# ascentai/diy-gym

Hardware: AMD Instinct MI355X
Metric: env steps/sec (whole node) (higher is better)
Workload: dtype f32; 1 GPU; ur_high_5 x 16384 envs per GPU; envs_total=16384, substeps=2, auto_reset=True, launch=hipGraph replay of 8-step segments, parallelism=independent env shards x1, no collective, envs_per_wavefront=64, lds_bytes_per_workgroup=160512, parity=vs the C oracle only; parity with pybullet itself is UNPINNED (DESIGN.md 4)

## Files before the change

### diy_gym_amd/csrc/dg_kernels.h

```cpp
#pragma once
#include "dg_device.h"
#include "../../include/diygym_scene.h"
#include "../../include/diygym_hip.h"

namespace dg {

#define DG_MAX_LINKS 64
#define DG_MAX_BODIES 192

#define DG_CONSTANT __attribute__((address_space(4)))
typedef const int32_t DG_CONSTANT* cip;
typedef const float DG_CONSTANT* cfp;

struct DevScene {
  cip BI, LI, FI, SI, PI, GI, OI, IL;
  cfp BF, LF, FF, SF, PF, OF, FL, HF;
  cip PLB;
  int split_pgs;
  int early_dyn;
  int coll_split, cont2_off;
  int coll_wave;
  cfp GD;
  cip AM;
  cip SD;
// ... 17 lines not shown
  int32_t reg_body[2];
  int32_t num_envs, stride;
  uint64_t seed; int64_t env_base;
  float h, gx, gy, gz;
  float hm;
};
struct MotorTable { float v[DG_MAX_LINKS * 3]; };

enum { PLB_R0 = 0, PLB_MINV, PLB_DV, PLB_NV, PLB_CHAIN , PLB_STRIDE };
enum { PLL_POSE = 0, PLL_MROW, PLL_IAACC , PLL_STRIDE };
enum { AW_E = 0, AW_R = 9, AW_V = 12, AW_PA = 18, AW_U = 24, AW_D = 30, AW_UU = 31, AW_STRIDE = 32 };
enum { AB_V = 0, AB_A = 6, AB_FIXED_STRIDE = 12, AB_IA = 12, AB_PA = 33, AB_L = 39, AB_FLOAT_STRIDE = 60 };
enum { CL_PAIR = 0, CL_P = 1, CL_N = 4, CL_DIST = 7, CL_KEY = 8, CL_DVA = 9, CL_NVA = 10, CL_DVB = 11, CL_NVB = 12, CL_MU = 13, CL_STRIDE = 14 };
enum { MR_B = 0, MR_ACC, MR_LO_B, MR_LO_ACC, MR_HI_B, MR_HI_ACC, MR_STRIDE };

constexpr int envs_per_wave(int lanes) { return lanes > 0 ? lanes : (lanes < 0 ? -lanes : 64); }

template <int LANES>
DGD float* workspace_of(const DevScene& sc, float* smem, float* gws, int lane) {
  if constexpr (LANES > 0) return smem + lane;
  else return gws + (size_t)blockIdx.x * (size_t)sc.total_slots * envs_per_wave(LANES) + lane;
}

template <int LANES>
struct Lane {
  const DevScene& sc;
  const MotorTable& mt;
  float* lds;
  float* st;
  int env;
  bool valid;

  DGD Lane(const DevScene& s, const MotorTable& m, float* l, float* state, int e, bool v) : sc(s), mt(m), lds(l), st(state), env(e), valid(v) {}

  DGD float& L(int slot) const { return lds[slot * envs_per_wave(LANES)]; }
  DGD float S(int k) const { return st[(size_t)k * sc.stride]; }
  DGD void Sset(int k, float v) const { if (valid) st[(size_t)k * sc.stride] = v; }

  DGD V3 L3(int o) const { return v3(L(o), L(o + 1), L(o + 2)); }
  DGD void L3set(int o, V3 v) const { L(o) = v.x; L(o + 1) = v.y; L(o + 2) = v.z; }
  DGD M3 LM(int o) const { M3 A; _Pragma("unroll") for (int k = 0; k < 9; k++) A.m[k] = L(o + k); return A; }
  DGD void LMset(int o, const M3& A) const { _Pragma("unroll") for (int k = 0; k < 9; k++) L(o + k) = A.m[k]; }
  DGD M3 LR(int o) const {
    V3 c0 = v3(L(o), L(o + 1), L(o + 2)), c1 = v3(L(o + 3), L(o + 4), L(o + 5)), c2 = cross(c0, c1);
    M3 R = {{c0.x, c1.x, c2.x, c0.y, c1.y, c2.y, c0.z, c1.z, c2.z}}; return R;
  }
// ... 37 lines not shown
  DGD V3 base_pos(int b) const {
    if (frozen(b)) { cfp f = bf(b) + DG_BF_INIT_POS; return v3(f[0], f[1], f[2]); }
    int o = bi(b)[DG_BI_STATE_OFF]; return v3(S(o), S(o + 1), S(o + 2));
  }
  DGD Q4 base_quat(int b) const {
    if (frozen(b)) { cfp f = bf(b) + DG_BF_INIT_QUAT; Q4 q = {f[0], f[1], f[2], f[3]}; return q; }
    int o = bi(b)[DG_BI_STATE_OFF] + DG_BS_QUAT; Q4 q = {S(o), S(o + 1), S(o + 2), S(o + 3)}; return q;
  }

  DGD void link_world(int b, int gl, M3& R, V3& p) const {
    if (gl < 0) { R = frozen(b) ? qmat(base_quat(b)) : LR(plb(b)[PLB_R0]); p = base_pos(b); }
    else { int o = pll(gl)[PLL_POSE]; R = LR(o); p = L3(o + 6); }
  }

  DGD void joint_xform(int gl, float q, M3& Rpc, V3& r) const {
    cfp f = lf(gl);
    M3 RT; _Pragma("unroll") for (int k = 0; k < 9; k++) RT.m[k] = f[DG_LF_ROT + k];
    V3 pT = v3(f[DG_LF_POS], f[DG_LF_POS + 1], f[DG_LF_POS + 2]);
    V3 ax = v3(f[DG_LF_AXIS], f[DG_LF_AXIS + 1], f[DG_LF_AXIS + 2]);
    if (li(gl)[DG_LI_TYPE] == 0) { Rpc = mul(RT, rot_axis(ax, q)); r = pT; }
    else { Rpc = RT; r = pT + mul(RT, ax * q); }
  }

  DGD void kinematics_chain(int b) const {
    constexpr int N = 6;
    cip B = bi(b); const int first = B[DG_BI_FIRST_LINK], n = B[DG_BI_N_LINKS];
    M3 R = qmat(base_quat(b)); V3 p = base_pos(b);
    LRset(plb(b)[PLB_R0], R);
    float qv[N];
#pragma unroll
    for (int j = 0; j < N; j++) qv[j] = S(li(first + min(j, n - 1))[DG_LI_STATE_OFF] + DG_LS_Q);
#pragma unroll
    for (int j = 0; j < N; j++) {
      if (j < n) {
        const int gl = first + j; M3 Rpc; V3 r; joint_xform(gl, qv[j], Rpc, r);
        const M3 Rn = mul(R, Rpc); p = p + mul(R, r);
        const int o = pll(gl)[PLL_POSE];
        LRset(o, Rn); L3set(o + 6, p);
        const V3 c0 = v3(Rn.m[0], Rn.m[3], Rn.m[6]), c1 = v3(Rn.m[1], Rn.m[4], Rn.m[7]), c2 = cross(c0, c1);
        const M3 Rb = {{c0.x, c1.x, c2.x, c0.y, c1.y, c2.y, c0.z, c1.z, c2.z}}; R = Rb;
      }
    }
  }
  DGD void kinematics(int b, int qoff = -1) const {
    cip B = bi(b);
    if (B[DG_BI_FLAGS] & DG_BODY_FROZEN) return;
    if (qoff < 0 && plb(b)[PLB_CHAIN]) { kinematics_chain(b); return; }
    int first = B[DG_BI_FIRST_LINK], n = B[DG_BI_N_LINKS];
    M3 R0 = qmat(base_quat(b)); V3 p0 = base_pos(b);
    LRset(plb(b)[PLB_R0], R0);
    constexpr int KCH = 8;
    for (int i0 = 0; i0 < n; i0 += KCH) {
      float qv[KCH];
#pragma unroll
      for (int j = 0; j < KCH; j++) { const int i = min(i0 + j, n - 1); qv[j] = qoff >= 0 ? L(qoff + i) : S(li(first + i)[DG_LI_STATE_OFF] + DG_LS_Q); }
#pragma unroll
      for (int j = 0; j < KCH; j++) {
        const int i = i0 + j; if (i >= n) break;
        int gl = first + i, par = li(gl)[DG_LI_PARENT];
        M3 Rpc; V3 r; joint_xform(gl, qv[j], Rpc, r);
        M3 Rp; V3 pp;
        if (par < 0) { Rp = R0; pp = p0; } else { int o = pll(par)[PLL_POSE]; Rp = LR(o); pp = L3(o + 6); }
        int o = pll(gl)[PLL_POSE];
        LRset(o, mul(Rp, Rpc)); L3set(o + 6, pp + mul(Rp, r));
// ... 191 lines not shown
        float rhs[6] = {-p0.a.x, -p0.a.y, -p0.a.z, -p0.l.x, -p0.l.y, -p0.l.z}, x[6];
        if (jdof < 0) {
#pragma unroll
          for (int k = 0; k < 6; k++) rhs[k] = (k == col) ? 1.0f : 0.0f;
        }
        chol6_solve(Lb, rhs, x);
        a0c.a = v3(x[0], x[1], x[2]); a0c.l = v3(x[3], x[4], x[5]);
#pragma unroll
        for (int k = 0; k < 6; k++) L(mo + col * nv + k) = x[k];
      }
      for (int i = 0; i <= jdof; i++) {
        int gl = first + i, par = li(gl)[DG_LI_PARENT]; int o = aw(i);
        S6 ap = par < 0 ? a0c : L6(aw(par - first) + AW_V);
        S6 a1 = xmotion(LM(o + AW_E), L3(o + AW_R), ap);
        float qdd = (L(o + AW_UU) - dot(L6(o + AW_U), a1)) / L(o + AW_D);
        L6set(o + AW_V, a1 + subspace(gl) * qdd);
        L(mo + col * nv + nb6 + i) = qdd;
      }
    }
    for (int r = 0; r < nv; r++) for (int c = r + 1; c < nv; c++) L(mo + r * nv + c) = L(mo + c * nv + r);
    prof.stamp(4 );
  }

  template <int N, class PROF_T>
  DGD void dynamics_chain(int b, PROF_T& prof) const {
    cip B = bi(b); const int first = B[DG_BI_FIRST_LINK], n = B[DG_BI_N_LINKS], mo = plb(b)[PLB_MINV]; const float h = sc.h;
    const M3 R0 = LR(plb(b)[PLB_R0]); const V3 gb = tmul(R0, v3(sc.gx, sc.gy, sc.gz));
    const float ka = ang_damping(b);
    const S6 zero6 = {v3(0.f, 0.f, 0.f), v3(0.f, 0.f, 0.f)};
    M3 E[N]; V3 r[N]; S6 v[N], pA[N], U[N], Sx[N]; float dinv[N], u[N], qd[N];
    S6 vp = zero6;
#pragma unroll
    for (int i = 0; i < N; i++) {
      E[i] = R0; r[i] = v3(0.f, 0.f, 0.f); v[i] = zero6; pA[i] = zero6; U[i] = zero6; Sx[i] = zero6; dinv[i] = 0.f; u[i] = 0.f; qd[i] = 0.f;
      if (i < n) {
        const int gl = first + i, lo = li(gl)[DG_LI_STATE_OFF]; cfp f = lf(gl);
        const float q = S(lo + DG_LS_Q); qd[i] = S(lo + DG_LS_QD);
        M3 Rpc; joint_xform(gl, q, Rpc, r[i]); E[i] = transpose(Rpc); Sx[i] = subspace(gl);
        v[i] = xmotion(E[i], r[i], vp) + Sx[i] * qd[i]; vp = v[i];
        float lm; V3 c; Sym3 Ic; link_inertia(gl, lm, c, Ic); (void)f;
        const AI I = rigid_inertia(lm, c, Ic);
        pA[i] = crf(v[i], mul(I, v[i])) - damping_force(lm, c, Ic, v[i], ka);
      }
    }
    AI carry; bool have = false;
#pragma unroll
    for (int i = N - 1; i >= 0; i--) {
      if (i < n) {
        const int gl = first + i, lo = li(gl)[DG_LI_STATE_OFF]; cfp f = lf(gl);
        const float tau = S(lo + DG_LS_TORQUE) - f[DG_LF_DAMPING] * qd[i];
        AI IA; { float lm; V3 lc; Sym3 lI; link_inertia(gl, lm, lc, lI); IA = rigid_inertia(lm, lc, lI); }
        if (have) {
          IA.I.xx += carry.I.xx; IA.I.xy += carry.I.xy; IA.I.xz += carry.I.xz; IA.I.yy += carry.I.yy; IA.I.yz += carry.I.yz; IA.I.zz += carry.I.zz;
          IA.M.xx += carry.M.xx; IA.M.xy += carry.M.xy; IA.M.xz += carry.M.xz; IA.M.yy += carry.M.yy; IA.M.yz += carry.M.yz; IA.M.zz += carry.M.zz;
#pragma unroll
          for (int k = 0; k < 9; k++) IA.H.m[k] += carry.H.m[k];
        }
        U[i] = mul(IA, Sx[i]); const float d = dot(Sx[i], U[i]); dinv[i] = 1.0f / d; u[i] = tau - dot(Sx[i], pA[i]);
        if (i > 0) {
          const float di = dinv[i]; const S6 Ui = U[i];
          AI Ia = IA;
          Ia.I.xx -= Ui.a.x * Ui.a.x * di; Ia.I.xy -= Ui.a.x * Ui.a.y * di; Ia.I.xz -= Ui.a.x * Ui.a.z * di;
          Ia.I.yy -= Ui.a.y * Ui.a.y * di; Ia.I.yz -= Ui.a.y * Ui.a.z * di; Ia.I.zz -= Ui.a.z * Ui.a.z * di;
          Ia.M.xx -= Ui.l.x * Ui.l.x * di; Ia.M.xy -= Ui.l.x * Ui.l.y * di; Ia.M.xz -= Ui.l.x * Ui.l.z * di;
          Ia.M.yy -= Ui.l.y * Ui.l.y * di; Ia.M.yz -= Ui.l.y * Ui.l.z * di; Ia.M.zz -= Ui.l.z * Ui.l.z * di;
          const float ua[3] = {Ui.a.x, Ui.a.y, Ui.a.z}, ul[3] = {Ui.l.x, Ui.l.y, Ui.l.z};
#pragma unroll
          for (int a = 0; a < 3; a++)
#pragma unroll
            for (int c2 = 0; c2 < 3; c2++) Ia.H.m[3 * a + c2] -= ua[a] * ul[c2] * di;
          const S6 c = crm(v[i], Sx[i] * qd[i]);
          const S6 pa = pA[i] + mul(Ia, c) + Ui * (u[i] * di);
          carry = to_parent(Ia, E[i], r[i]); have = true;
          pA[i - 1] = pA[i - 1] + xforce_to_parent(E[i], r[i], pa);
        }
      }
    }
    S6 ap; ap.a = v3(0.f, 0.f, 0.f); ap.l = -gb;
#pragma unroll
    for (int i = 0; i < N; i++) {
      if (i < n) {
        const S6 a1 = xmotion(E[i], r[i], ap) + crm(v[i], Sx[i] * qd[i]);
        const float qdd = (u[i] - dot(U[i], a1)) * dinv[i];
        ap = a1 + Sx[i] * qdd;
        Sset(li(first + i)[DG_LI_STATE_OFF] + DG_LS_QD, qd[i] + h * qdd);
      }
    }
    prof.stamp(3 );
#pragma unroll
    for (int col = 0; col < N; col++) {
      if (col < n) {
        S6 p[N]; float uu[N];
#pragma unroll
        for (int i = 0; i < N; i++) { p[i] = zero6; uu[i] = 0.f; }
#pragma unroll
        for (int i = col; i >= 0; i--) {
          uu[i] = (i == col ? 1.0f : 0.0f) - dot(Sx[i], p[i]);
          if (i > 0) p[i - 1] = p[i - 1] + xforce_to_parent(E[i], r[i], p[i] + U[i] * (uu[i] * dinv[i]));
        }
        S6 a = zero6;
#pragma unroll
        for (int i = 0; i < N; i++) {
          if (i < n) {
            const S6 a1 = xmotion(E[i], r[i], a);
            const float qdd = (uu[i] - dot(U[i], a1)) * dinv[i];
            a = a1 + Sx[i] * qdd;
            L(mo + col * n + i) = qdd;
          }
// ... 142 lines not shown
```

### diy_gym_amd/csrc/dg_solver.h

```cpp
#pragma once
#include "dg_kernels.h"
#include "dg_hull.h"

namespace dg {

enum { PS_UPDATE = 0, PS_KIN, PS_COLLIDE, PS_ABA, PS_MINV, PS_ROWS, PS_PGS, PS_INTEGRATE, PS_OUTPUT, PS_PGS_MOTOR, PS_PGS_LIMIT, PS_PGS_CONTACT, PS_COUNT,
       PS_ROW = PS_COUNT + 12  };
template <bool PROF> struct Prof;
template <> struct Prof<false> { DGD void start() {} DGD void stamp(int) {} };
template <> struct Prof<true> {
  unsigned long long last, acc[PS_COUNT];
  DGD void start() { _Pragma("unroll") for (int k = 0; k < PS_COUNT; k++) acc[k] = 0ull; last = __builtin_amdgcn_s_memtime(); }
  DGD void stamp(int id) {
    unsigned long long t = __builtin_amdgcn_s_memtime();
    _Pragma("unroll") for (int k = 0; k < PS_COUNT; k++) if (k == id) acc[k] += t - last;
    last = t;
  }
};

struct WShape { int type, body, glink; M3 R; V3 p; float prm0, prm1, prm2, mu; int poff, npts; };

template <int LANES>
DGD void shape_world(const Lane<LANES>& ln, int sh, WShape& o) {
  cip si = ln.sc.SI + sh * DG_SI_STRIDE; cfp sf = ln.sc.SF + sh * DG_SF_STRIDE;
// ... 1548 lines not shown
              const float mu = buf[d].mu;
              if (mu > 0.f) { const float lim = mu * buf[d].nacc; solve_row(buf[d], 3 * (t >> 1) + 1 + (t & 1), -lim, lim); }
            }
          }
        }
      }
    }
    prof.stamp(PS_PGS_CONTACT);
    if (live) iters_done = it + 1;
    live = live && !(maxres <= thr);
    if (!__any(live)) break;
  }
#pragma unroll
  for (int i = 0; i < NS; i++) if (i * SL + sl < nt) blk[(unsigned)(sc.dv_base + i * SL) * W + (lane_off >> 2)] = dv[i];
  if (sl == 0) for (int c = 0; c < ncont; c++) { _Pragma("unroll") for (int d = 0; d < 3; d++) blk[(unsigned)(r0 + (3 * c + d) * rs + 2 * nt + 1) * W + colq] = acc[(3 * c + d) * EPW]; }
  for (uint64_t m = rows.motors; m; m &= m - 1) {
    const int gl = __ffsll((long long)m) - 1; int col, mo, jg, base, nv; float lm; rows.get(gl, col, mo, jg, base, nv, lm);
    blk[(unsigned)(mo + MR_ACC) * W + colq] = acc[(3 * maxc + gl) * EPW];
  }
  return __shfl(iters_done, (lane << LOG) & 63);
}

template <int LANES>
DGD void setup_link_rows(const Lane<LANES>& ln, int g0, int g1, uint64_t& limit_mask, uint64_t& limit_rows) {
  const DevScene& sc = ln.sc; const float h = sc.h, lerp = sc.HF[DG_HF_LIMIT_ERP];
  constexpr int LCH = 6;
  for (int gc = g0; gc < g1; gc += LCH) {
    float q_[LCH], qd_[LCH], tp_[LCH], tv_[LCH];
#pragma unroll
    for (int j = 0; j < LCH; j++) {
      const int gl = min(gc + j, g1 - 1), lo = ln.li(gl)[DG_LI_STATE_OFF];
      q_[j] = ln.S(lo + DG_LS_Q); qd_[j] = ln.S(lo + DG_LS_QD); tp_[j] = ln.S(lo + DG_LS_TARGET_POS); tv_[j] = ln.S(lo + DG_LS_TARGET_VEL);
    }
#pragma unroll
    for (int j = 0; j < LCH; j++) {
      const int gl = gc + j; if (gl >= g1) break;
      const int mo = ln.pll(gl)[PLL_MROW]; cfp f = ln.lf(gl);
      const float q = q_[j], qd = qd_[j];
      const float kp = ln.mt.v[3 * gl], kd = ln.mt.v[3 * gl + 1];
      ln.L(mo + MR_B) = kp * (tp_[j] - q) / h + kd * (tv_[j] - qd);
      ln.L(mo + MR_ACC) = 0.f;
      const bool limited = f[DG_LF_LOWER] <= f[DG_LF_UPPER];
      const float dlo = q - f[DG_LF_LOWER], dhi = f[DG_LF_UPPER] - q;
      ln.L(mo + MR_LO_B) = -qd + (dlo > 0.f ? -dlo / h : -dlo * lerp / h); ln.L(mo + MR_LO_ACC) = (limited && dlo < 0.25f) ? 0.f : -1.f;
      ln.L(mo + MR_HI_B) = qd + (dhi > 0.f ? -dhi / h : -dhi * lerp / h); ln.L(mo + MR_HI_ACC) = (limited && dhi < 0.25f) ? 0.f : -1.f;
      if (__any(limited && (dlo < 0.25f || dhi < 0.25f))) limit_mask |= 1ull << (ln.li(gl)[DG_LI_BODY] & 63);
      if (gl < 32) { if (__any(limited && dlo < 0.25f)) limit_rows |= 1ull << (2 * gl); if (__any(limited && dhi < 0.25f)) limit_rows |= 2ull << (2 * gl); }
    }
  }
}

template <int LANES>
DGD void integrate_body(const Lane<LANES>& ln, int b) {
  const DevScene& sc = ln.sc; const float h = sc.h, vmax = sc.HF[DG_HF_MAX_COORD_VEL];
  constexpr int LCH = 6;
  cip B = ln.bi(b); const int n = B[DG_BI_N_LINKS], first = B[DG_BI_FIRST_LINK], so = B[DG_BI_STATE_OFF];
  const bool fx = ln.fixed(b); if (fx && n == 0) return;
  const int dvo = ln.plb(b)[PLB_DV];
  if (!fx) {
    M3 R0 = ln.LR(ln.plb(b)[PLB_R0]);
    V3 dw = mul(R0, ln.L3(dvo)), dl = mul(R0, ln.L3(dvo + 3));
    V3 w = v3(ln.S(so + DG_BS_ANGVEL), ln.S(so + DG_BS_ANGVEL + 1), ln.S(so + DG_BS_ANGVEL + 2)) + dw;
    V3 v = v3(ln.S(so + DG_BS_LINVEL), ln.S(so + DG_BS_LINVEL + 1), ln.S(so + DG_BS_LINVEL + 2)) + dl;
    ln.Sset(so + DG_BS_ANGVEL, w.x); ln.Sset(so + DG_BS_ANGVEL + 1, w.y); ln.Sset(so + DG_BS_ANGVEL + 2, w.z);
    ln.Sset(so + DG_BS_LINVEL, v.x); ln.Sset(so + DG_BS_LINVEL + 1, v.y); ln.Sset(so + DG_BS_LINVEL + 2, v.z);
    ln.Sset(so, ln.S(so) + h * v.x); ln.Sset(so + 1, ln.S(so + 1) + h * v.y); ln.Sset(so + 2, ln.S(so + 2) + h * v.z);
    float wn = norm(w), th = wn * h; Q4 dq;
    if (th > 1e-12f) { float sn, cs; sincosf(0.5f * th, &sn, &cs); sn /= wn; dq.x = w.x * sn; dq.y = w.y * sn; dq.z = w.z * sn; dq.w = cs; }
    else { dq.x = 0.5f * h * w.x; dq.y = 0.5f * h * w.y; dq.z = 0.5f * h * w.z; dq.w = 1.f; }
    Q4 qn = qnormalize(qmul(dq, ln.base_quat(b)));
    ln.Sset(so + 3, qn.x); ln.Sset(so + 4, qn.y); ln.Sset(so + 5, qn.z); ln.Sset(so + 6, qn.w);
  }
  const int k0 = fx ? 0 : 6;
  for (int i0 = 0; i0 < n; i0 += LCH) {
    float q_[LCH], qd_[LCH], dv_[LCH], ac_[LCH]; int lo_[LCH];
#pragma unroll
    for (int j = 0; j < LCH; j++) {
      const int i = min(i0 + j, n - 1); lo_[j] = ln.li(first + i)[DG_LI_STATE_OFF];
      q_[j] = ln.S(lo_[j] + DG_LS_Q); qd_[j] = ln.S(lo_[j] + DG_LS_QD); dv_[j] = ln.L(dvo + k0 + i); ac_[j] = ln.L(ln.pll(first + i)[PLL_MROW] + MR_ACC);
    }
#pragma unroll
    for (int j = 0; j < LCH; j++) {
      const int i = i0 + j; if (i >= n) break;
      const float maxf = ln.mt.v[3 * (first + i) + 2]; const float maximp = maxf < 0.f ? -maxf : maxf * sc.hm;
      ln.Sset(lo_[j] + DG_LS_APPLIED, maximp > 0.f ? ac_[j] / h : 0.f);
      const float qd = fminf(fmaxf(qd_[j] + dv_[j], -vmax), vmax);
      ln.Sset(lo_[j] + DG_LS_QD, qd); ln.Sset(lo_[j] + DG_LS_Q, q_[j] + h * qd);
    }
  }
}

#define DG_SPLIT_MAX_CONTACTS 3
DGD int split_slots(const DevScene& sc) { return sc.dv_base + sc.nt + sc.nv_max; }

template <int LANES>
DGD bool split_decide_main(const Lane<LANES>& ln, int wave_max_cont, uint64_t& limit_mask, uint64_t& limit_rows) {
  const DevScene& sc = ln.sc; const int xo = split_slots(sc);
  ln.L(xo + 4) = (sc.split_pgs && (wave_max_cont == 0 || (sc.split_pgs == 2 && wave_max_cont <= DG_SPLIT_MAX_CONTACTS))) ? 1.f : 0.f;
  __syncthreads();
  const unsigned hbits = (unsigned)ln.L(xo + 5);
  if (hbits) { limit_mask |= 1ull << (sc.helper_body & 63); limit_rows |= (uint64_t)hbits << (2 * ln.bi(sc.helper_body)[DG_BI_FIRST_LINK]); }
  return ln.L(xo + 4) != 0.f;
}
template <int LANES>
DGD bool split_decide_follow(const Lane<LANES>& ln, unsigned my_limit_bits, bool i_am_helper) {
  const DevScene& sc = ln.sc; const int xo = split_slots(sc);
  if (i_am_helper) ln.L(xo + 5) = (float)my_limit_bits;
  __syncthreads();
  return ln.L(xo + 4) != 0.f;
}

DGD float half_swap_max(float x) {
  float a = x, b = x;
  asm volatile("s_nop 1\n\tv_permlane32_swap_b32 %0, %1" : "+v"(a), "+v"(b));
// ... 125 lines not shown
        contact_row(3 * c + 1, -lim, lim, lv, maxabs); contact_row(3 * c + 2, -lim, lim, lv, maxabs);
      }
    }
    const float m = half_swap_max(maxabs);
    live = live && !(m <= thr_abs);
  };
  if (cmax > 0) {
    for (int it = 0; it < sc.iters; it++) { if (live) iters_done = it + 1; sweep(std::true_type{}, std::true_type{}); if (!__any(live)) break; }
  } else if (lim_rows == 0u) {
    for (int it = 0; it < sc.iters; it++) { if (live) iters_done = it + 1; sweep(std::false_type{}, std::false_type{}); if (!__any(live)) break; }
  } else {
    for (int it = 0; it < sc.iters; it++) { if (live) iters_done = it + 1; sweep(std::true_type{}, std::false_type{}); if (!__any(live)) break; }
  }
#pragma unroll
  for (int i = 0; i < RN; i++) if (i < n) { W(dvo + i) = rdv[i]; W(mo0 + i * MR_STRIDE + MR_ACC) = racc[i]; }
  if (cmax > 0 && half == 0) {
    const int rs = sc.crow_tail + 3;
#pragma unroll
    for (int c = 0; c < CM; c++) if (c < ncont) { _Pragma("unroll") for (int d = 0; d < 3; d++) W(sc.tr_off + (3 * c + d) * rs + sc.crow_tail + 1) = cacc[3 * c + d]; }
  }
  if (half == 0) W(split_slots(sc)) = (float)iters_done;
}

template <int LANES, bool PROF, bool PAR = false, bool SLICED = false, bool FULLWAVE = false>
DGD void substep(const Lane<LANES>& ln, int32_t* diag_out, Prof<PROF>& prof, float* smem = nullptr, float* gws = nullptr, int index = 0) {
  const DevScene& sc = ln.sc; const float h = sc.h; const int hb = PAR ? sc.helper_body : -1;
  const bool primary = SLICED ? (int)threadIdx.x < envs_per_wave(LANES) : true;
  constexpr int LCH = 6;
  int ncont = 0, wave_max_cont = 0, iters_done = 0;
  uint64_t limit_mask = 0ull;
  uint64_t limit_rows = 0ull;
  const float thr = sc.HF[DG_HF_RESIDUAL_THRESHOLD]; const int rs = crow_stride(sc.crow_tail);
  const bool early = PAR && sc.early_dyn && index == 0;
  constexpr int EPW = envs_per_wave(LANES), SLN = SLICED ? 64 / EPW : 1, SLOG = SLN == 64 ? 6 : SLN == 16 ? 4 : SLN == 8 ? 3 : SLN == 4 ? 2 : SLN == 2 ? 1 : 0;
  const int qlane = threadIdx.x & 63, qsl = qlane & (SLN - 1), qe = qlane >> SLOG;
  const int qenv = blockIdx.x * EPW + qe; const bool qvalid = qenv < sc.num_envs; const int qec = qvalid ? qenv : sc.num_envs - 1;
  const Lane<LANES> lq(sc, ln.mt, SLICED ? ln.lds - qlane + qe : ln.lds, SLICED ? ln.st - ln.env + qec : ln.st, SLICED ? qec : ln.env, SLICED ? qvalid : ln.valid);
  if (primary) {
  if (index == sc.substeps - 1 && !early) for (int b = 0; b < sc.nba; b++) if (b != hb) save_prev_velocities(ln, b);
  if (!early) for (int b = 0; b < sc.nba; b++) if (b != hb) ln.kinematics(b);
  }
  if (PAR) __syncthreads();
  prof.stamp(PS_KIN);
  if constexpr (SLICED) collide<LANES, 64, SLN>(lq, 0, 0x7fffffff, -1, qsl);
  const bool own_collide = !(PAR && sc.coll_wave);
  if (primary) {
  if constexpr (SLICED) ncont = (int)ln.L(sc.cont_off);
  else if (own_collide) ncont = collide<LANES, FULLWAVE ? 64 : (PAR ? 64 : 0)>(ln);
  prof.stamp(PS_COLLIDE);
  }
  if (!early) for (int b = 0; b < sc.nba; b++) {
    if (b == hb || (ln.fixed(b) && ln.bi(b)[DG_BI_N_LINKS] == 0)) continue;
    const int mslices = (SLICED && !ln.plb(b)[PLB_CHAIN] && !sc.no_minv_slices) ? ln.minv_slices(b, SLN) : 0;
    if (primary) { if (ln.plb(b)[PLB_CHAIN]) ln.template dynamics_chain<6>(b, prof); else ln.dynamics(b, prof, mslices > 0); }
    if constexpr (SLICED) { if (mslices > 0) { lq.minv_sliced(b, qsl, mslices, SLN); prof.stamp(4 ); } }
    if (primary) {
      const int dvo = ln.plb(b)[PLB_DV], nv = ln.plb(b)[PLB_NV];
      for (int k = 0; k < nv; k++) ln.L(dvo + k) = 0.f;
    }
  }
  if (primary) {
  if (PAR) __syncthreads();
  if (!own_collide) {
    ncont = (int)ln.L(sc.cont_off);
    if (sc.coll_split) {
      const int nb2 = (int)ln.L(sc.cont2_off);
      if (__any(nb2 > 0)) {
        for (int j = 0; j < sc.max_contacts; j++) {
          if (!__any(j < nb2)) break;
          if (j < nb2 && ncont + j < sc.max_contacts) {
            float* dst = ln.lds + (sc.cont_off + 1 + (ncont + j) * CL_STRIDE) * envs_per_wave(LANES);
#pragma unroll
            for (int k = 0; k < CL_KEY + 1; k++) dst[k * envs_per_wave(LANES)] = ln.L(sc.cont2_off + 1 + j * CL_STRIDE + k);
          }
        }
        ncont = min(ncont + nb2, sc.max_contacts); ln.L(sc.cont_off) = (float)ncont;
      }
    }
  }
  const bool helper_rows = PAR && sc.split_pgs;
  if (helper_rows) {
    const int hf = ln.bi(hb)[DG_BI_FIRST_LINK], hn = ln.bi(hb)[DG_BI_N_LINKS];
    setup_link_rows(ln, 0, hf, limit_mask, limit_rows); setup_link_rows(ln, hf + hn, sc.nl, limit_mask, limit_rows);
  } else setup_link_rows(ln, 0, sc.nl, limit_mask, limit_rows);
  for (int b = 0; b < sc.nba; b++) {
    if (ln.bi(b)[DG_BI_N_LINKS] == 0 || b == sc.reg_body[0] || b == sc.reg_body[1] || (helper_rows && b == hb)) continue;
    motor_guess(ln, b);
  }
  if (sc.ncons > 0) build_constraint_rows(ln);
  const bool vel_dense = sc.dense && sc.nt >= 1 && sc.reg_body[0] < 0;
  wave_max_cont = [&] { int m = ncont; for (int o = 32; o > 0; o >>= 1) m = max(m, __shfl_xor(m, o)); return m; }();
  if (vel_dense && wave_max_cont > 0)
    for (int b = 0; b < sc.nba; b++) if (!(ln.fixed(b) && ln.bi(b)[DG_BI_N_LINKS] == 0)) ln.gen_vel_store(b, ln.plb(b)[PLB_DV]);
  if constexpr (!SLICED) {
  for (int c = 0; c < wave_max_cont; c++) {
    const bool has = c < ncont; const int mypair = has ? (int)ln.L(sc.cont_off + 1 + c * CL_STRIDE + CL_PAIR) : -1;
    bool todo = has && !build_contact_rows_base(ln, c, has, vel_dense);
    if (!sc.no_chain_rows) todo = todo && !build_contact_rows_chains(ln, c, todo);
    while (__any(todo)) {
      const int leader = __ffsll((long long)__ballot(todo)) - 1;
      const int pair = __shfl(mypair, leader);
      const bool mine = todo && mypair == pair;
      build_contact_rows(ln, c, pair, mine, vel_dense);
      todo = todo && !mine;
// ... 190 lines not shown
    live = live && !(maxres <= thr && maxabs <= thr_abs);
    if (!__any(live)) break;
  }
#pragma unroll
  for (int k = 0; k < NBR; k++) {
    const int b = sc.reg_body[k];
    if (b >= 0) {
      regs_to_lds(k);
      const int mo0 = ln.pll(ln.bi(b)[DG_BI_FIRST_LINK])[PLL_MROW];
#pragma unroll
      for (int i = 0; i < RN; i++) if (i < rn[k]) ln.L(mo0 + i * MR_STRIDE + MR_ACC) = racc[k][i];
    }
  }
  }
  }
  prof.stamp(PS_PGS);
  if (primary) {
  store_warm_cache(ln, ncont, wave_max_cont);
  if (diag_out && ln.valid) {
    int32_t* d = diag_out + (size_t)DG_DIAG_STRIDE * ln.env;
    d[DG_DIAG_CONTACTS] = ncont; d[DG_DIAG_PGS_ITERS] = iters_done;
    if (index == 0) { d[DG_DIAG_PGS_ITERS_FIRST] = iters_done; d[DG_DIAG_CONTACTS_FIRST] = ncont; }
  }
  for (int b = 0; b < sc.nba; b++) if (!(split_now && b == hb)) integrate_body(ln, b);
  }
  if (PAR) __syncthreads();
}

template <int LANES>
DGD void helper_substep(const Lane<LANES>& ln, bool early, bool last) {
  const DevScene& sc = ln.sc; const int hb = sc.helper_body; Prof<false> none;
  if (last && !early) save_prev_velocities(ln, hb);
  if (!early) ln.kinematics(hb);
  __syncthreads();
  if (!early) {
    ln.template dynamics_chain<6>(hb, none);
    const int dvo = ln.plb(hb)[PLB_DV], nv = ln.plb(hb)[PLB_NV]; for (int k = 0; k < nv; k++) ln.L(dvo + k) = 0.f;
  }
  __syncthreads();
  uint64_t lm = 0ull, lr = 0ull;
  if (sc.split_pgs) { const int hf = ln.bi(hb)[DG_BI_FIRST_LINK]; setup_link_rows(ln, hf, hf + ln.bi(hb)[DG_BI_N_LINKS], lm, lr); }
  const int hf0 = ln.bi(hb)[DG_BI_FIRST_LINK];
  if (split_decide_follow(ln, hf0 + 6 <= 32 ? (unsigned)((lr >> (2 * hf0)) & 0xFFFull) : 0u, true)) {
    pgs_reg_halves(ln, 1);
    __syncthreads();
    integrate_body(ln, hb);
  }
  __syncthreads();
}

template <int LANES, bool PROF, bool PAR = false, bool SLICED = false, bool FULLWAVE = false>
DGD void sim_step(const Lane<LANES>& ln, int32_t* diag_out, Prof<PROF>& prof, float* smem = nullptr, float* gws = nullptr) {
  const DevScene& sc = ln.sc;
  for (int k = 0; k < sc.substeps; k++) { substep<LANES, PROF, PAR, SLICED, FULLWAVE>(ln, diag_out, prof, smem, gws, k); prof.stamp(PS_INTEGRATE); }
  if (SLICED && (int)threadIdx.x >= envs_per_wave(LANES)) return;
  if (sc.debug_keep_ext) return;
  for (int b = 0; b < sc.nba; b++) { if (ln.frozen(b)) continue; const int eo = ln.ext_off(b); for (int k = 0; k < 6; k++) ln.Sset(eo + k, 0.f); }
  for (int gl = 0; gl < sc.nl; gl++) ln.Sset(ln.li(gl)[DG_LI_STATE_OFF] + DG_LS_TORQUE, 0.f);
}

template <int LANES>
DGD int run_ik(const Lane<LANES>& ln, int op, const float* act, bool live_lane) {
  const DevScene& sc = ln.sc; cip oi = sc.OI + op * DG_OI_STRIDE;
  const int b = oi[DG_OI_BODY], fr = oi[DG_OI_FRAME], flags = oi[DG_OI_FLAGS];
  const bool use_orn = flags & DG_IK_USE_ORIENTATION, nullsp = flags & DG_IK_NULLSPACE;
  const int first = ln.bi(b)[DG_BI_FIRST_LINK], n = ln.bi(b)[DG_BI_N_LINKS];
  const int qo = sc.tr_off, jo = qo + n, vo = jo + 6 * n, dto = vo + n;
  cfp rest = sc.FL + oi[DG_OI_FLIST];
  for (int i = 0; i < n; i++) ln.L(qo + i) = ln.S(ln.li(first + i)[DG_LI_STATE_OFF] + DG_LS_Q);
  V3 cp, cv, cw; Q4 cq; ln.frame_state(b, fr, true, cp, cq, cv, cw, false);
  V3 tp = cp + v3(act[0], act[1], act[2]); Q4 tq = cq;
  if (use_orn) tq = qmul(cq, qfrom_euler(act[3], act[4], act[5]));
  const int eel = sc.FI[fr * DG_FI_STRIDE + DG_FI_LINK];
  const float lam2 = nullsp ? sc.HF[DG_HF_IK_LAMBDA_SQ] : sc.HF[DG_HF_IK_JOINT_DAMPING], maxang = sc.HF[DG_HF_IK_MAX_ANGLE], g0 = sc.HF[DG_HF_IK_NULL_REST_GAIN], g1 = sc.HF[DG_HF_IK_NULL_LIMIT_GAIN];
  const float resid = sc.HF[DG_HF_IK_RESIDUAL];
  bool live = live_lane; int iters = 0;
  for (int it = 0; it < sc.ik_iters; it++) {
// ... 727 lines not shown
```

### diy_gym_amd/csrc/dg_step_par_body.inc

```
  constexpr int reset_mode = DG_PAR_RESET;
  extern __shared__ float smem[];
  const int wave = threadIdx.x >> 6, lane = threadIdx.x & 63;
  const int env = blockIdx.x * 64 + lane; const bool exists = env < sc.num_envs; const int e = exists ? env : sc.num_envs - 1;
  const bool doit = exists && (!reset_mode || reset_mask == nullptr || reset_mask[e] != 0);
  if (reset_mode && !__any(doit)) return;
  const bool valid = reset_mode ? doit : exists;
  const float* act_row = actions ? actions + (size_t)e * sc.act_dim : nullptr;
  const unsigned long long t_start = PROF ? __builtin_amdgcn_s_memtime() : 0ull; (void)t_start;
  if (wave == 3) {
    Lane<64> ln(sc, mt, smem + lane, state + e, e, valid);
    if (reset_mode) __syncthreads();
    DG_WAVE_STAMP(0); __syncthreads();
    if (sc.early_dyn) {
      early_dynamics(ln, 1);
      if (sc.coll_split) collide<64, 64>(ln, sc.npairs / 2, 0x7fffffff, sc.cont2_off);
    }
    DG_WAVE_STAMP(1); __syncthreads();
    for (int k = 0; k < sc.substeps; k++) {
      __syncthreads();
      if (sc.coll_split && !(sc.early_dyn && k == 0)) collide<64, 64>(ln, sc.npairs / 2, 0x7fffffff, sc.cont2_off);
      __syncthreads();
      if (split_decide_follow(ln, 0u, false)) __syncthreads();
      __syncthreads();
    }
// ... 11 lines not shown
      collide<64, 64>(ln, 0, sc.coll_split ? sc.npairs / 2 : 0x7fffffff);
      early_dynamics(ln, 0);
    }
    DG_WAVE_STAMP(1); __syncthreads();
    for (int k = 0; k < sc.substeps; k++) {
      __syncthreads();
      if (sc.coll_wave && !(sc.early_dyn && k == 0)) collide<64, 64>(ln, 0, sc.coll_split ? sc.npairs / 2 : 0x7fffffff);
      __syncthreads();
      if (split_decide_follow(ln, false, false)) __syncthreads();
      __syncthreads();
    }
    DG_WAVE_STAMP(2); __syncthreads();
    run_output_ops(ln, (valid && obs) ? obs + (size_t)e * sc.obs_dim : nullptr, nullptr, nullptr, nullptr, nullptr, OUT_OBS_REST);
    DG_WAVE_STAMP(3);
    return;
  }
  if (wave == 1) {
    Lane<64> ln(sc, mt, smem + lane, state + e, e, valid);
    if (reset_mode) __syncthreads();
    ln.kinematics(sc.helper_body);
    DG_WAVE_STAMP(0); __syncthreads();
    if (act_row) run_update_ops(ln, act_row, mask, sc.helper_body, -1, diag);
    DG_WAVE_STAMP(1); __syncthreads();
    for (int k = 0; k < sc.substeps; k++) helper_substep(ln, sc.early_dyn && k == 0, k == sc.substeps - 1);
    ln.kinematics(sc.helper_body);
    DG_WAVE_STAMP(2); __syncthreads();
    run_output_ops(ln, (valid && obs) ? obs + (size_t)e * sc.obs_dim : nullptr, nullptr, nullptr, nullptr, nullptr, OUT_JOINT_OF, sc.helper_body);
    DG_WAVE_STAMP(3);
    return;
  }
  Lane<64> ln(sc, mt, smem + lane, state + e, e, valid);
  Prof<PROF> prof; prof.start();
  if (reset_mode) { if (doit) { ln.Sset(DG_ST_STEP, 0.0f); run_reset_ops(ln); } __syncthreads(); }
  for (int b = 0; b < sc.nba; b++) if (b != sc.helper_body) ln.kinematics(b);
  __syncthreads();
  prof.stamp(PS_KIN);
  if (act_row) run_update_ops(ln, act_row, mask, -1, sc.helper_body, diag);
  if (!reset_mode) ln.Sset(DG_ST_STEP, ln.S(DG_ST_STEP) + 1.0f);
  __syncthreads();
  prof.stamp(PS_UPDATE);
  sim_step<64, PROF, true>(ln, diag, prof);
  for (int b = 0; b < sc.nba; b++) if (b != sc.helper_body) ln.kinematics(b);
  __syncthreads();
  prof.stamp(PS_KIN);
  run_output_ops(ln, (valid && obs) ? obs + (size_t)e * sc.obs_dim : nullptr, nullptr, nullptr, nullptr, nullptr, OUT_JOINT_NOT_OF, sc.helper_body);
  prof.stamp(PS_OUTPUT);
  if constexpr (PROF) { if (lane == 0) for (int k = 0; k < PS_COUNT; k++) cycles[(size_t)blockIdx.x * PS_ROW + k] = prof.acc[k]; }
```

Baseline: 170.6 million env-steps/s.

## Carry chain-body joint state in registers across substeps instead of reloading from global

```diff
diff --git a/diy_gym_amd/csrc/dg_kernels.h b/diy_gym_amd/csrc/dg_kernels.h
--- a/diy_gym_amd/csrc/dg_kernels.h
+++ b/diy_gym_amd/csrc/dg_kernels.h
@@ -63,6 +63,13 @@
   else return gws + (size_t)blockIdx.x * (size_t)sc.total_slots * envs_per_wave(LANES) + lane;
 }
 
+struct ChainRegs {
+  bool on;
+  float q[6], qd[6], tp[6], tv[6], tq[6];
+  Q4 bq; V3 bp;
+  M3 Rpc[6]; V3 r[6];
+};
+
 template <int LANES>
 struct Lane {
   const DevScene& sc;
@@ -146,24 +153,51 @@
     else { Rpc = RT; r = pT + mul(RT, ax * q); }
   }
 
-  DGD void kinematics_chain(int b) const {
+  template <bool CR = false>
+  DGD void kinematics_chain(int b, ChainRegs* c = nullptr) const {
     constexpr int N = 6;
     cip B = bi(b); const int first = B[DG_BI_FIRST_LINK], n = B[DG_BI_N_LINKS];
-    M3 R = qmat(base_quat(b)); V3 p = base_pos(b);
+    bool on = false; if constexpr (CR) on = c->on;
+    M3 R; V3 p; float qv[N];
+    if constexpr (CR) { if (on) {
+      R = qmat(c->bq); p = c->bp;
+#pragma unroll
+      for (int j = 0; j < N; j++) qv[j] = c->q[j];
+    } }
+    if (!on) {
+      R = qmat(base_quat(b)); p = base_pos(b);
+#pragma unroll
+      for (int j = 0; j < N; j++) qv[j] = S(li(first + min(j, n - 1))[DG_LI_STATE_OFF] + DG_LS_Q);
+    }
     LRset(plb(b)[PLB_R0], R);
-    float qv[N];
-#pragma unroll
-    for (int j = 0; j < N; j++) qv[j] = S(li(first + min(j, n - 1))[DG_LI_STATE_OFF] + DG_LS_Q);
 #pragma unroll
     for (int j = 0; j < N; j++) {
       if (j < n) {
         const int gl = first + j; M3 Rpc; V3 r; joint_xform(gl, qv[j], Rpc, r);
+        if constexpr (CR) { c->Rpc[j] = Rpc; c->r[j] = r; }
         const M3 Rn = mul(R, Rpc); p = p + mul(R, r);
         const int o = pll(gl)[PLL_POSE];
         LRset(o, Rn); L3set(o + 6, p);
         const V3 c0 = v3(Rn.m[0], Rn.m[3], Rn.m[6]), c1 = v3(Rn.m[1], Rn.m[4], Rn.m[7]), c2 = cross(c0, c1);
         const M3 Rb = {{c0.x, c1.x, c2.x, c0.y, c1.y, c2.y, c0.z, c1.z, c2.z}}; R = Rb;
       }
+    }
+  }
+  DGD void chain_load(int b, ChainRegs& c) const {
+    cip B = bi(b); const int first = B[DG_BI_FIRST_LINK], n = B[DG_BI_N_LINKS];
+    c.bq = base_quat(b); c.bp = base_pos(b);
+#pragma unroll
+    for (int j = 0; j < 6; j++) {
+      const int lo = li(first + min(j, n - 1))[DG_LI_STATE_OFF];
+      c.q[j] = S(lo + DG_LS_Q); c.qd[j] = S(lo + DG_LS_QD); c.tp[j] = S(lo + DG_LS_TARGET_POS); c.tv[j] = S(lo + DG_LS_TARGET_VEL); c.tq[j] = S(lo + DG_LS_TORQUE);
+    }
+  }
+  DGD void chain_reload(int b, ChainRegs& c, bool with_q) const {
+    cip B = bi(b); const int first = B[DG_BI_FIRST_LINK], n = B[DG_BI_N_LINKS];
+#pragma unroll
+    for (int j = 0; j < 6; j++) {
+      const int lo = li(first + min(j, n - 1))[DG_LI_STATE_OFF];
+      c.qd[j] = S(lo + DG_LS_QD); if (with_q) c.q[j] = S(lo + DG_LS_Q);
     }
   }
   DGD void kinematics(int b, int qoff = -1) const {
@@ -401,8 +435,9 @@
     prof.stamp(4 );
   }
 
-  template <int N, class PROF_T>
-  DGD void dynamics_chain(int b, PROF_T& prof) const {
+  template <int N, bool CR = false, class PROF_T>
+  DGD void dynamics_chain(int b, PROF_T& prof, ChainRegs* c = nullptr) const {
+    bool on = false; if constexpr (CR) on = c->on;
     cip B = bi(b); const int first = B[DG_BI_FIRST_LINK], n = B[DG_BI_N_LINKS], mo = plb(b)[PLB_MINV]; const float h = sc.h;
     const M3 R0 = LR(plb(b)[PLB_R0]); const V3 gb = tmul(R0, v3(sc.gx, sc.gy, sc.gz));
     const float ka = ang_damping(b);
@@ -414,8 +449,9 @@
       E[i] = R0; r[i] = v3(0.f, 0.f, 0.f); v[i] = zero6; pA[i] = zero6; U[i] = zero6; Sx[i] = zero6; dinv[i] = 0.f; u[i] = 0.f; qd[i] = 0.f;
       if (i < n) {
         const int gl = first + i, lo = li(gl)[DG_LI_STATE_OFF]; cfp f = lf(gl);
-        const float q = S(lo + DG_LS_Q); qd[i] = S(lo + DG_LS_QD);
-        M3 Rpc; joint_xform(gl, q, Rpc, r[i]); E[i] = transpose(Rpc); Sx[i] = subspace(gl);
+        if constexpr (CR) { if (on) { qd[i] = c->qd[i]; E[i] = transpose(c->Rpc[i]); r[i] = c->r[i]; } }
+        if (!on) { const float q = S(lo + DG_LS_Q); qd[i] = S(lo + DG_LS_QD); M3 Rpc; joint_xform(gl, q, Rpc, r[i]); E[i] = transpose(Rpc); }
+        Sx[i] = subspace(gl);
         v[i] = xmotion(E[i], r[i], vp) + Sx[i] * qd[i]; vp = v[i];
         float lm; V3 c; Sym3 Ic; link_inertia(gl, lm, c, Ic); (void)f;
         const AI I = rigid_inertia(lm, c, Ic);
@@ -427,7 +463,9 @@
     for (int i = N - 1; i >= 0; i--) {
       if (i < n) {
         const int gl = first + i, lo = li(gl)[DG_LI_STATE_OFF]; cfp f = lf(gl);
-        const float tau = S(lo + DG_LS_TORQUE) - f[DG_LF_DAMPING] * qd[i];
+        float tq = 0.f; if constexpr (CR) { if (on) tq = c->tq[i]; }
+        if (!on) tq = S(lo + DG_LS_TORQUE);
+        const float tau = tq - f[DG_LF_DAMPING] * qd[i];
         AI IA; { float lm; V3 lc; Sym3 lI; link_inertia(gl, lm, lc, lI); IA = rigid_inertia(lm, lc, lI); }
         if (have) {
           IA.I.xx += carry.I.xx; IA.I.xy += carry.I.xy; IA.I.xz += carry.I.xz; IA.I.yy += carry.I.yy; IA.I.yz += carry.I.yz; IA.I.zz += carry.I.zz;
@@ -462,7 +500,9 @@
         const S6 a1 = xmotion(E[i], r[i], ap) + crm(v[i], Sx[i] * qd[i]);
         const float qdd = (u[i] - dot(U[i], a1)) * dinv[i];
         ap = a1 + Sx[i] * qdd;
-        Sset(li(first + i)[DG_LI_STATE_OFF] + DG_LS_QD, qd[i] + h * qdd);
+        const float qdn = qd[i] + h * qdd;
+        Sset(li(first + i)[DG_LI_STATE_OFF] + DG_LS_QD, qdn);
+        if constexpr (CR) c->qd[i] = qdn;
       }
     }
     prof.stamp(3 );
diff --git a/diy_gym_amd/csrc/dg_solver.h b/diy_gym_amd/csrc/dg_solver.h
--- a/diy_gym_amd/csrc/dg_solver.h
+++ b/diy_gym_amd/csrc/dg_solver.h
@@ -1594,8 +1594,21 @@
 }
 
 template <int LANES>
+DGD void link_rows(const Lane<LANES>& ln, int gl, float q, float qd, float tp, float tv, uint64_t& limit_mask, uint64_t& limit_rows) {
+  const DevScene& sc = ln.sc; const float h = sc.h, lerp = sc.HF[DG_HF_LIMIT_ERP];
+  const int mo = ln.pll(gl)[PLL_MROW]; cfp f = ln.lf(gl);
+  const float kp = ln.mt.v[3 * gl], kd = ln.mt.v[3 * gl + 1];
+  ln.L(mo + MR_B) = kp * (tp - q) / h + kd * (tv - qd);
+  ln.L(mo + MR_ACC) = 0.f;
+  const bool limited = f[DG_LF_LOWER] <= f[DG_LF_UPPER];
+  const float dlo = q - f[DG_LF_LOWER], dhi = f[DG_LF_UPPER] - q;
+  ln.L(mo + MR_LO_B) = -qd + (dlo > 0.f ? -dlo / h : -dlo * lerp / h); ln.L(mo + MR_LO_ACC) = (limited && dlo < 0.25f) ? 0.f : -1.f;
+  ln.L(mo + MR_HI_B) = qd + (dhi > 0.f ? -dhi / h : -dhi * lerp / h); ln.L(mo + MR_HI_ACC) = (limited && dhi < 0.25f) ? 0.f : -1.f;
+  if (__any(limited && (dlo < 0.25f || dhi < 0.25f))) limit_mask |= 1ull << (ln.li(gl)[DG_LI_BODY] & 63);
+  if (gl < 32) { if (__any(limited && dlo < 0.25f)) limit_rows |= 1ull << (2 * gl); if (__any(limited && dhi < 0.25f)) limit_rows |= 2ull << (2 * gl); }
+}
+template <int LANES>
 DGD void setup_link_rows(const Lane<LANES>& ln, int g0, int g1, uint64_t& limit_mask, uint64_t& limit_rows) {
-  const DevScene& sc = ln.sc; const float h = sc.h, lerp = sc.HF[DG_HF_LIMIT_ERP];
   constexpr int LCH = 6;
   for (int gc = g0; gc < g1; gc += LCH) {
     float q_[LCH], qd_[LCH], tp_[LCH], tv_[LCH];
@@ -1607,19 +1620,15 @@
 #pragma unroll
     for (int j = 0; j < LCH; j++) {
       const int gl = gc + j; if (gl >= g1) break;
-      const int mo = ln.pll(gl)[PLL_MROW]; cfp f = ln.lf(gl);
-      const float q = q_[j], qd = qd_[j];
-      const float kp = ln.mt.v[3 * gl], kd = ln.mt.v[3 * gl + 1];
-      ln.L(mo + MR_B) = kp * (tp_[j] - q) / h + kd * (tv_[j] - qd);
-      ln.L(mo + MR_ACC) = 0.f;
-      const bool limited = f[DG_LF_LOWER] <= f[DG_LF_UPPER];
-      const float dlo = q - f[DG_LF_LOWER], dhi = f[DG_LF_UPPER] - q;
-      ln.L(mo + MR_LO_B) = -qd + (dlo > 0.f ? -dlo / h : -dlo * lerp / h); ln.L(mo + MR_LO_ACC) = (limited && dlo < 0.25f) ? 0.f : -1.f;
-      ln.L(mo + MR_HI_B) = qd + (dhi > 0.f ? -dhi / h : -dhi * lerp / h); ln.L(mo + MR_HI_ACC) = (limited && dhi < 0.25f) ? 0.f : -1.f;
-      if (__any(limited && (dlo < 0.25f || dhi < 0.25f))) limit_mask |= 1ull << (ln.li(gl)[DG_LI_BODY] & 63);
-      if (gl < 32) { if (__any(limited && dlo < 0.25f)) limit_rows |= 1ull << (2 * gl); if (__any(limited && dhi < 0.25f)) limit_rows |= 2ull << (2 * gl); }
-    }
-  }
+      link_rows(ln, gl, q_[j], qd_[j], tp_[j], tv_[j], limit_mask, limit_rows);
+    }
+  }
+}
+template <int LANES>
+DGD void setup_chain_rows(const Lane<LANES>& ln, int b, const ChainRegs& c, uint64_t& limit_mask, uint64_t& limit_rows) {
+  const int first = ln.bi(b)[DG_BI_FIRST_LINK], n = ln.bi(b)[DG_BI_N_LINKS];
+#pragma unroll
+  for (int j = 0; j < 6; j++) if (j < n) link_rows(ln, first + j, c.q[j], c.qd[j], c.tp[j], c.tv[j], limit_mask, limit_rows);
 }
 
 template <int LANES>
@@ -1662,6 +1671,28 @@
   }
 }
 
+template <int LANES>
+DGD void integrate_chain(const Lane<LANES>& ln, int b, ChainRegs& c) {
+  const DevScene& sc = ln.sc; const float h = sc.h, vmax = sc.HF[DG_HF_MAX_COORD_VEL];
+  cip B = ln.bi(b); const int n = B[DG_BI_N_LINKS], first = B[DG_BI_FIRST_LINK];
+  const int dvo = ln.plb(b)[PLB_DV];
+  float dv_[6], ac_[6];
+#pragma unroll
+  for (int j = 0; j < 6; j++) { const int i = min(j, n - 1); dv_[j] = ln.L(dvo + i); ac_[j] = ln.L(ln.pll(first + i)[PLL_MROW] + MR_ACC); }
+#pragma unroll
+  for (int j = 0; j < 6; j++) {
+    if (j < n) {
+      const int lo = ln.li(first + j)[DG_LI_STATE_OFF];
+      const float maxf = ln.mt.v[3 * (first + j) + 2]; const float maximp = maxf < 0.f ? -maxf : maxf * sc.hm;
+      ln.Sset(lo + DG_LS_APPLIED, maximp > 0.f ? ac_[j] / h : 0.f);
+      const float qd = fminf(fmaxf(c.qd[j] + dv_[j], -vmax), vmax);
+      const float qn = c.q[j] + h * qd;
+      ln.Sset(lo + DG_LS_QD, qd); ln.Sset(lo + DG_LS_Q, qn);
+      c.qd[j] = qd; c.q[j] = qn;
+    }
+  }
+}
+
 #define DG_SPLIT_MAX_CONTACTS 3
 DGD int split_slots(const DevScene& sc) { return sc.dv_base + sc.nt + sc.nv_max; }
 
@@ -1833,9 +1864,17 @@
   if (half == 0) W(split_slots(sc)) = (float)iters_done;
 }
 
+template <int LANES>
+DGD bool chain_carry(const Lane<LANES>& ln) {
+  const DevScene& sc = ln.sc;
+  return sc.split_pgs > 0 && ln.plb(sc.reg_body[0])[PLB_CHAIN] != 0 && ln.plb(sc.helper_body)[PLB_CHAIN] != 0;
+}
+
 template <int LANES, bool PROF, bool PAR = false, bool SLICED = false, bool FULLWAVE = false>
-DGD void substep(const Lane<LANES>& ln, int32_t* diag_out, Prof<PROF>& prof, float* smem = nullptr, float* gws = nullptr, int index = 0) {
+DGD void substep(const Lane<LANES>& ln, int32_t* diag_out, Prof<PROF>& prof, float* smem = nullptr, float* gws = nullptr, int index = 0, ChainRegs* cr = nullptr) {
   const DevScene& sc = ln.sc; const float h = sc.h; const int hb = PAR ? sc.helper_body : -1;
+  bool carry = false; int cb = -1;
+  if constexpr (PAR) { carry = cr->on; cb = carry ? sc.reg_body[0] : -1; }
   const bool primary = SLICED ? (int)threadIdx.x < envs_per_wave(LANES) : true;
   constexpr int LCH = 6;
   int ncont = 0, wave_max_cont = 0, iters_done = 0;
@@ -1849,7 +1888,10 @@
   const Lane<LANES> lq(sc, ln.mt, SLICED ? ln.lds - qlane + qe : ln.lds, SLICED ? ln.st - ln.env + qec : ln.st, SLICED ? qec : ln.env, SLICED ? qvalid : ln.valid);
   if (primary) {
   if (index == sc.substeps - 1 && !early) for (int b = 0; b < sc.nba; b++) if (b != hb) save_prev_velocities(ln, b);
-  if (!early) for (int b = 0; b < sc.nba; b++) if (b != hb) ln.kinematics(b);
+  if (!early) for (int b = 0; b < sc.nba; b++) if (b != hb) {
+    if constexpr (PAR) { if (b == cb) { ln.template kinematics_chain<true>(b, cr); continue; } }
+    ln.kinematics(b);
+  }
   }
   if (PAR) __syncthreads();
   prof.stamp(PS_KIN);
@@ -1863,7 +1905,12 @@
   if (!early) for (int b = 0; b < sc.nba; b++) {
     if (b == hb || (ln.fixed(b) && ln.bi(b)[DG_BI_N_LINKS] == 0)) continue;
     const int mslices = (SLICED && !ln.plb(b)[PLB_CHAIN] && !sc.no_minv_slices) ? ln.minv_slices(b, SLN) : 0;
-    if (primary) { if (ln.plb(b)[PLB_CHAIN]) ln.template dynamics_chain<6>(b, prof); else ln.dynamics(b, prof, mslices > 0); }
+    if (primary) {
+      bool done = false;
+      if constexpr (PAR) { if (b == cb) { ln.template dynamics_chain<6, true>(b, prof, cr); done = true; } }
+      if (done) {}
+      else if (ln.plb(b)[PLB_CHAIN]) ln.template dynamics_chain<6>(b, prof); else ln.dynamics(b, prof, mslices > 0);
+    }
     if constexpr (SLICED) { if (mslices > 0) { lq.minv_sliced(b, qsl, mslices, SLN); prof.stamp(4 ); } }
     if (primary) {
       const int dvo = ln.plb(b)[PLB_DV], nv = ln.plb(b)[PLB_NV];
@@ -1872,6 +1919,7 @@
   }
   if (primary) {
   if (PAR) __syncthreads();
+  if constexpr (PAR) { if (carry && early) ln.chain_reload(cb, *cr, false); }
   if (!own_collide) {
     ncont = (int)ln.L(sc.cont_off);
     if (sc.coll_split) {
@@ -1890,7 +1938,10 @@
     }
   }
   const bool helper_rows = PAR && sc.split_pgs;
-  if (helper_rows) {
+  bool rows_done = false;
+  if constexpr (PAR) { if (carry) { setup_chain_rows(ln, cb, *cr, limit_mask, limit_rows); rows_done = true; } }
+  if (rows_done) {}
+  else if (helper_rows) {
     const int hf = ln.bi(hb)[DG_BI_FIRST_LINK], hn = ln.bi(hb)[DG_BI_N_LINKS];
     setup_link_rows(ln, 0, hf, limit_mask, limit_rows); setup_link_rows(ln, hf + hn, sc.nl, limit_mask, limit_rows);
   } else setup_link_rows(ln, 0, sc.nl, limit_mask, limit_rows);
@@ -2127,37 +2178,44 @@
     d[DG_DIAG_CONTACTS] = ncont; d[DG_DIAG_PGS_ITERS] = iters_done;
     if (index == 0) { d[DG_DIAG_PGS_ITERS_FIRST] = iters_done; d[DG_DIAG_CONTACTS_FIRST] = ncont; }
   }
-  for (int b = 0; b < sc.nba; b++) if (!(split_now && b == hb)) integrate_body(ln, b);
+  for (int b = 0; b < sc.nba; b++) if (!(split_now && b == hb)) {
+    if constexpr (PAR) { if (b == cb) { integrate_chain(ln, b, *cr); continue; } }
+    integrate_body(ln, b);
+  }
   }
   if (PAR) __syncthreads();
 }
 
 template <int LANES>
-DGD void helper_substep(const Lane<LANES>& ln, bool early, bool last) {
+DGD void helper_substep(const Lane<LANES>& ln, bool early, bool last, ChainRegs& cr) {
   const DevScene& sc = ln.sc; const int hb = sc.helper_body; Prof<false> none;
   if (last && !early) save_prev_velocities(ln, hb);
-  if (!early) ln.kinematics(hb);
+  if (!early) { if (cr.on) ln.template kinematics_chain<true>(hb, &cr); else ln.kinematics(hb); }
   __syncthreads();
   if (!early) {
-    ln.template dynamics_chain<6>(hb, none);
+    ln.template dynamics_chain<6, true>(hb, none, &cr);
     const int dvo = ln.plb(hb)[PLB_DV], nv = ln.plb(hb)[PLB_NV]; for (int k = 0; k < nv; k++) ln.L(dvo + k) = 0.f;
   }
   __syncthreads();
+  if (cr.on && early) ln.chain_reload(hb, cr, false);
   uint64_t lm = 0ull, lr = 0ull;
-  if (sc.split_pgs) { const int hf = ln.bi(hb)[DG_BI_FIRST_LINK]; setup_link_rows(ln, hf, hf + ln.bi(hb)[DG_BI_N_LINKS], lm, lr); }
+  if (cr.on) setup_chain_rows(ln, hb, cr, lm, lr);
+  else if (sc.split_pgs) { const int hf = ln.bi(hb)[DG_BI_FIRST_LINK]; setup_link_rows(ln, hf, hf + ln.bi(hb)[DG_BI_N_LINKS], lm, lr); }
   const int hf0 = ln.bi(hb)[DG_BI_FIRST_LINK];
-  if (split_decide_follow(ln, hf0 + 6 <= 32 ? (unsigned)((lr >> (2 * hf0)) & 0xFFFull) : 0u, true)) {
+  const bool split_now = split_decide_follow(ln, hf0 + 6 <= 32 ? (unsigned)((lr >> (2 * hf0)) & 0xFFFull) : 0u, true);
+  if (split_now) {
     pgs_reg_halves(ln, 1);
     __syncthreads();
-    integrate_body(ln, hb);
+    if (cr.on) integrate_chain(ln, hb, cr); else integrate_body(ln, hb);
   }
   __syncthreads();
+  if (cr.on && !split_now) ln.chain_reload(hb, cr, true);
 }
 
 template <int LANES, bool PROF, bool PAR = false, bool SLICED = false, bool FULLWAVE = false>
-DGD void sim_step(const Lane<LANES>& ln, int32_t* diag_out, Prof<PROF>& prof, float* smem = nullptr, float* gws = nullptr) {
+DGD void sim_step(const Lane<LANES>& ln, int32_t* diag_out, Prof<PROF>& prof, float* smem = nullptr, float* gws = nullptr, ChainRegs* cr = nullptr) {
   const DevScene& sc = ln.sc;
-  for (int k = 0; k < sc.substeps; k++) { substep<LANES, PROF, PAR, SLICED, FULLWAVE>(ln, diag_out, prof, smem, gws, k); prof.stamp(PS_INTEGRATE); }
+  for (int k = 0; k < sc.substeps; k++) { substep<LANES, PROF, PAR, SLICED, FULLWAVE>(ln, diag_out, prof, smem, gws, k, cr); prof.stamp(PS_INTEGRATE); }
   if (SLICED && (int)threadIdx.x >= envs_per_wave(LANES)) return;
   if (sc.debug_keep_ext) return;
   for (int b = 0; b < sc.nba; b++) { if (ln.frozen(b)) continue; const int eo = ln.ext_off(b); for (int k = 0; k < 6; k++) ln.Sset(eo + k, 0.f); }
diff --git a/diy_gym_amd/csrc/dg_step_par_body.inc b/diy_gym_amd/csrc/dg_step_par_body.inc
--- a/diy_gym_amd/csrc/dg_step_par_body.inc
+++ b/diy_gym_amd/csrc/dg_step_par_body.inc
@@ -57,8 +57,10 @@
     DG_WAVE_STAMP(0); __syncthreads();
     if (act_row) run_update_ops(ln, act_row, mask, sc.helper_body, -1, diag);
     DG_WAVE_STAMP(1); __syncthreads();
-    for (int k = 0; k < sc.substeps; k++) helper_substep(ln, sc.early_dyn && k == 0, k == sc.substeps - 1);
-    ln.kinematics(sc.helper_body);
+    ChainRegs cr; cr.on = chain_carry(ln);
+    if (cr.on) ln.chain_load(sc.helper_body, cr);
+    for (int k = 0; k < sc.substeps; k++) helper_substep(ln, sc.early_dyn && k == 0, k == sc.substeps - 1, cr);
+    if (cr.on) ln.template kinematics_chain<true>(sc.helper_body, &cr); else ln.kinematics(sc.helper_body);
     DG_WAVE_STAMP(2); __syncthreads();
     run_output_ops(ln, (valid && obs) ? obs + (size_t)e * sc.obs_dim : nullptr, nullptr, nullptr, nullptr, nullptr, OUT_JOINT_OF, sc.helper_body);
     DG_WAVE_STAMP(3);
@@ -74,8 +76,10 @@
   if (!reset_mode) ln.Sset(DG_ST_STEP, ln.S(DG_ST_STEP) + 1.0f);
   __syncthreads();
   prof.stamp(PS_UPDATE);
-  sim_step<64, PROF, true>(ln, diag, prof);
-  for (int b = 0; b < sc.nba; b++) if (b != sc.helper_body) ln.kinematics(b);
+  ChainRegs cr; cr.on = chain_carry(ln);
+  if (cr.on) ln.chain_load(sc.reg_body[0], cr);
+  sim_step<64, PROF, true>(ln, diag, prof, nullptr, nullptr, &cr);
+  for (int b = 0; b < sc.nba; b++) if (b != sc.helper_body) { if (cr.on && b == sc.reg_body[0]) ln.template kinematics_chain<true>(b, &cr); else ln.kinematics(b); }
   __syncthreads();
   prof.stamp(PS_KIN);
   run_output_ops(ln, (valid && obs) ? obs + (size_t)e * sc.obs_dim : nullptr, nullptr, nullptr, nullptr, nullptr, OUT_JOINT_NOT_OF, sc.helper_body);
```

After: 165.5 million env-steps/s. -3.0%, worse.
